# KorAP/Datok

Hardware: AMD Instinct MI355X
Metric: input MB/s tokenized, tokenizer_de.matok (higher is better)
Workload: dtype u32 table cells, u8 symbol codes; 1 GPU; tokenizer_de.matok, 4096 equal-length 4096 B synthetic German docs per batch (BASELINE.json configs[1]); table_layout=matrix: state-major fused u32 cells, docs_per_gpu=4096, doc_bytes=4096, parallelism=documents sharded over 1 GPU(s), no data-path collective, batches_in_flight=3, inputs=one per batch in flight (generator seeds 2, 3, 4 on rank 0)

## Files before the change

### datok_amd/csrc/dtk_walk.hip

```cpp
#include "dtk_walk_core.h"

struct ExactSink {
  DtkSymAt s;
  const uint8_t *txt;
  bool nl_rule, write;
  DtkCall *log;
  int32_t *rstart, *rend, *sent;
  uint32_t *bstart, *bend, *ttok, *tsent, *sbefore, *ts_end;
  uint32_t tok_n, sent_n, text_n;
  int32_t posC, last_rend;
  bool init, sentB;
  uint32_t n_tok, n_sent, n_text, n_sev, text_tok0, n_calls;
  uint32_t st;
  __device__ __forceinline__ void start() {
    posC = 0; last_rend = 0; init = true; sentB = true;
    n_tok = n_sent = n_text = n_sev = text_tok0 = n_calls = 0; st = 0;
  }
  __device__ __forceinline__ int32_t runes(uint32_t from, uint32_t to) const {
    return to > from ? (int32_t)count_runes(s, from, to) : 0;
  }
  __device__ __forceinline__ void call(uint32_t kind, int32_t a, uint32_t b, uint32_t c) {
    if (write) log[n_calls] = DtkCall{kind, a, b, c};
    n_calls++;
  }
  __device__ __forceinline__ void push_sent(int32_t v) {
    if (write) { if (n_sent < sent_n) sent[n_sent] = v; else st |= ST_INTERNAL; }
    n_sent++;
  }
  __device__ __forceinline__ void sentence_end(int32_t arg) {
    call(1u, arg, 0u, 0u);
    n_sev++;
    if (n_tok == text_tok0) st |= ST_EMPTY_TEXT; else push_sent(last_rend);
    sentB = true;
  }
  __device__ __forceinline__ void text_end(int32_t arg) {
    call(2u, arg, 0u, 0u);
    if (n_tok == text_tok0) st |= ST_EMPTY_TEXT;
    if (write) {
      if (n_text < text_n) {
        ttok[n_text] = n_tok; tsent[n_text] = n_sent;
        if (ts_end) ts_end[n_text] = n_sev;
      } else st |= ST_INTERNAL;
    }
    n_text++;
    sentB = true; posC = 0; text_tok0 = n_tok;
  }
  template <bool IS_MATRIX>
  __device__ __forceinline__ void token(uint32_t bs, uint32_t tp, uint32_t p, bool) {
    call(0u, (int32_t)bs, tp, p);
    const int32_t off_r = runes(bs, tp), len_r = runes(bs, p);
    if (posC == 0 && nl_rule && p > bs && txt[bs] == '\n' && !init) posC--;
    init = false;
    posC += off_r;
    const int32_t rs = posC;
    if (sentB) { sentB = false; push_sent(rs); }
    posC += len_r - off_r;
    last_rend = posC;
    if (write) {
      if (n_tok < tok_n) {
        if (rstart) { rstart[n_tok] = rs; rend[n_tok] = posC; }
        if (bstart) { bstart[n_tok] = tp < p ? tp : p; bend[n_tok] = p; }
        if (sbefore) sbefore[n_tok] = n_sev;
      } else st |= ST_INTERNAL;
    }
    n_tok++;
  }
  template <bool IS_MATRIX>
  __device__ __forceinline__ void eot(uint32_t bs, uint32_t p, bool with_sentence, bool) {
    const int32_t buffc = runes(bs, p);
    if (with_sentence) sentence_end(buffc);
    text_end(IS_MATRIX ? buffc : 0);
  }
  template <bool IS_MATRIX>
  __device__ __forceinline__ void sentence(uint32_t bs, uint32_t p, bool) {
    sentence_end(IS_MATRIX ? runes(bs, p) : 0);
  }
  template <bool IS_MATRIX>
  __device__ __forceinline__ void tail(uint32_t bs, uint32_t p, bool sentence_end_, bool text_end_, bool) {
    const int32_t arg = IS_MATRIX ? runes(bs, p) : 0;
    if (!sentence_end_) sentence_end(arg);
    if (!text_end_) text_end(arg);
  }
  __device__ __forceinline__ void out_of_order() {}
};

template <typename TRANS, bool IS_MATRIX>
__global__ __launch_bounds__(WAVE) void k_exact_doc(TRANS tr, DtkExactArgs X, uint32_t epsilon, uint32_t unknown,
                                                    uint32_t identity) {
  __shared__ uint16_t s_win[WAVE * DTK_WIN_ROW];
  uint16_t *win_row = s_win + threadIdx.x * DTK_WIN_ROW;
  const uint32_t i = blockIdx.x * WAVE + threadIdx.x;
  if (i >= X.n) return;
  const uint32_t d = X.docs[i];
  const uint64_t off = X.doc_off[d];
  const uint32_t len = (uint32_t)(X.doc_off[d + 1] - off);
  ExactSink sink;
  sink.s = DtkSymAt{X.sym, off}; sink.txt = X.text + off;
  sink.nl_rule = (X.flags & 16u) != 0; sink.write = X.pass != 0;
  sink.log = X.pass ? X.calls + X.call_off[i] : nullptr;
  const uint64_t t0 = X.tok_off[d], s0 = X.sent_off[d], x0 = X.text_off[d];
  sink.rstart = X.tok_rstart ? X.tok_rstart + t0 : nullptr; sink.rend = X.tok_rend ? X.tok_rend + t0 : nullptr;
  sink.bstart = X.tok_bstart ? X.tok_bstart + t0 : nullptr; sink.bend = X.tok_bend ? X.tok_bend + t0 : nullptr;
  sink.sbefore = X.tok_sbefore ? X.tok_sbefore + t0 : nullptr;
  sink.sent = X.sent + s0;
  sink.ttok = X.text_tok_end + x0; sink.tsent = X.text_sent_end + x0;
  sink.ts_end = X.text_s_end ? X.text_s_end + x0 : nullptr;
  sink.tok_n = (uint32_t)(X.tok_off[d + 1] - t0); sink.sent_n = (uint32_t)(X.sent_off[d + 1] - s0);
  sink.text_n = (uint32_t)(X.text_off[d + 1] - x0);
  sink.start();
  DtkLaneState init{0u, tr.start_state(), tr.start_aux(), 0u}, fin;
  uint32_t st = 0, steps = 0;
  walk_lane<TRANS, IS_MATRIX, MODE_DOC, ExactSink>(tr, X.sym, off, len, init, 0u, sink, epsilon, unknown, identity,
                                                   step_cap(X.step_factor, len), fin, st, steps, win_row);
  if (X.pass == 0) { X.n_calls[i] = sink.n_calls; return; }
  if (sink.n_tok != sink.tok_n || sink.n_sent != sink.sent_n || sink.n_text != sink.text_n) st |= ST_INTERNAL;
  X.status[d] = st | sink.st;
  if (X.doc_ns) X.doc_ns[d] = sink.n_sev;
}

template <typename TRANS, bool IS_MATRIX>
__global__ __launch_bounds__(WAVE) void k_walk_doc(TRANS tr, DtkWalkArgs A, uint32_t epsilon,
                                                   uint32_t unknown, uint32_t identity) {
  DTK_WINDOWS(TRANS, A.sym)
  const uint32_t d = blockIdx.x * WAVE + threadIdx.x;
  uint32_t steps = 0;
  if (d < A.n_docs) {
    const uint64_t off = A.doc_off[d];
    const uint32_t len = (uint32_t)(A.doc_off[d + 1] - off);
    EventSink sink;
    sink.init(A, off, d, 0u, 0xFFFFFFFFu);
    DtkLaneState init{0u, tr.start_state(), tr.start_aux(), 0u}, fin;
    uint32_t st;
    walk_any<TRANS, IS_MATRIX, MODE_DOC>(tr, A.sym, off, len, init, 0u, sink, epsilon, unknown,
                                          identity, step_cap(A.step_factor, len), fin, st, steps, win_row, s_lut);
    A.status[d] = st | sink.st;
    A.tok_cnt[d] = sink.c_tok; A.sent_cnt[d] = sink.c_sent; A.text_cnt[d] = sink.c_text;
  }
  add_steps(A.steps, steps);
}


#ifdef DTK_PROBE
__shared__ unsigned long long s_probe_mark;
__device__ unsigned long long g_phase[8];
extern "C" int dtk_phase_read(unsigned long long *out, int reset) {
  hipDeviceSynchronize();
  hipMemcpyFromSymbol(out, HIP_SYMBOL(g_phase), sizeof(g_phase));
  if (reset) { unsigned long long z[8] = {0}; hipMemcpyToSymbol(HIP_SYMBOL(g_phase), z, sizeof(z)); }
  return 0;
}
#endif

template <typename TRANS, bool IS_MATRIX>
__device__ __forceinline__ DtkLaneState start_record(const TRANS &tr, const DtkWalkArgs &A, const DtkSpecArgs &S,
                                                     uint32_t k, uint64_t off, uint32_t len, uint32_t epsilon,
                                                     uint32_t unknown, uint32_t identity, uint16_t *win_row,
                                                     const uint16_t *s_lut, uint32_t &steps) {
  DtkLaneState rec{0u, tr.start_state(), tr.start_aux(), 0u};
  if (k > 0) {
    const uint32_t kc = k * S.chunk;
    uint32_t sp = kc > S.warm ? kc - S.warm : 0u;
    if (sp > 0 && S.warm_extend && S.text) {
      const uint8_t *tx = S.text + off;
      auto load8 = [&](uint32_t q) -> uint64_t {
        if (off + q >= 16u) {
          const uint64_t a0 = reinterpret_cast<uint64_t>(tx + q) - 8u;
          const uint32_t sh = (uint32_t)(a0 & 3u) * 8u;
          const uint32_t *wp = reinterpret_cast<const uint32_t *>(a0 & ~3ull);
          const uint64_t lo64 = (uint64_t)wp[0] | ((uint64_t)wp[1] << 32);
          return sh ? (lo64 >> sh) | ((uint64_t)wp[2] << (64u - sh)) : lo64;
        }
        uint64_t w = 0;
        for (uint32_t k = 0; k < 8u; k++)
          if (q + k >= 8u) w |= (uint64_t)tx[q + k - 8u] << (8u * k);
        return w;
      };
      auto zb = [](uint64_t x) {
        return ~(((x & 0x7F7F7F7F7F7F7F7Full) + 0x7F7F7F7F7F7F7F7Full) | x) & 0x8080808080808080ull;
      };
      const uint32_t lim = sp > S.warm_extend ? sp - S.warm_extend : 0u;
      uint32_t q = sp;
      while (q > lim) {
        const uint64_t w = load8(q);
        uint64_t m = zb(w ^ 0x2020202020202020ull) | zb(w ^ 0x0A0A0A0A0A0A0A0Aull) |
                     zb(w ^ 0x0909090909090909ull) | zb(w ^ 0x0D0D0D0D0D0D0D0Dull);
        if (q < 8u) m &= ~0ull << ((8u - q) * 8u);
        if (m) {
          q = q - 8u + (7u - ((uint32_t)__clzll((long long)m) >> 3)) + 1u;
          break;
        }
        q = q >= 8u ? q - 8u : 0u;
      }
      if (q < lim) q = lim;
      sp = q;
      uint64_t wt[DTK_WARM_TAG / 8u];
#pragma unroll
      for (uint32_t i = 0; i < DTK_WARM_TAG / 8u; i++) wt[i] = sp > 8u * i ? load8(sp - 8u * i) : 0ull;
#pragma unroll
      for (uint32_t i = 0; i < DTK_WARM_TAG / 8u; i++) {
        const uint32_t qq = sp > 8u * i ? sp - 8u * i : 0u;
        uint64_t mo = zb(wt[i] ^ 0x3C3C3C3C3C3C3C3Cull), mc = zb(wt[i] ^ 0x3E3E3E3E3E3E3E3Eull);
        if (qq < 8u) { const uint64_t in = qq ? ~0ull << ((8u - qq) * 8u) : 0ull; mo &= in; mc &= in; }
        if (mo | mc) {
          if (mo > mc) sp = qq - 8u + (7u - ((uint32_t)__clzll((long long)mo) >> 3));
          break;
        }
      }
    }
#ifdef DTK_PROBE
    s_probe_mark = clock64();
#endif
    EventSink sink;
    sink.g = nullptr; sink.lds = (dtk_lds_u32 *)nullptr; sink.tailw = nullptr; sink.lw = 0; sink.lo = sink.hi = 0;
    uint32_t st;
    if (sp > 0) {
      while (sp < len && !dtk_sym_is_start(A.sym, off + sp)) sp++;
      DtkLaneState init{sp, tr.start_state(), tr.start_aux(), 0u};
      walk_any<TRANS, IS_MATRIX, MODE_START>(tr, A.sym, off, len, init, kc, sink, epsilon, unknown,
                                              identity, step_cap(A.step_factor, len), rec, st, steps, win_row, s_lut);
    } else {
      walk_any<TRANS, IS_MATRIX, MODE_START>(tr, A.sym, off, len, rec, kc, sink, epsilon, unknown,
                                              identity, step_cap(A.step_factor, len), rec, st, steps, win_row, s_lut);
    }
  }
  return rec;
}

template <typename TRANS, bool IS_MATRIX>
__global__ __launch_bounds__(WAVE) void k_spec_start(TRANS tr, DtkWalkArgs A, DtkSpecArgs S,
                                                     uint32_t epsilon, uint32_t unknown,
                                                     uint32_t identity) {
  DTK_WINDOWS(TRANS, A.sym)
  const uint32_t L = blockIdx.x * WAVE + threadIdx.x;
  uint32_t steps = 0;
  if (L < S.n_lanes) {
    const uint32_t d = S.lane_doc[L];
    const uint32_t k = L - S.chunk_off[d];
    const uint64_t off = A.doc_off[d];
    const uint32_t len = (uint32_t)(A.doc_off[d + 1] - off);
    S.lane_start[L] = start_record<TRANS, IS_MATRIX>(tr, A, S, k, off, len, epsilon, unknown, identity, win_row, s_lut, steps);
  }
  add_steps(A.steps, steps);
}

extern __shared__ uint32_t s_dyn_bits[];

#ifndef DTK_WALK_OCC
#define DTK_WALK_OCC 7
#endif
template <typename TRANS, bool IS_MATRIX>
__global__ __launch_bounds__(WAVE, TRANS::LEAN ? DTK_WALK_OCC : 1) void k_spec_both(TRANS tr, DtkWalkArgs A, DtkSpecArgs S,
                                                    uint32_t epsilon, uint32_t unknown,
                                                    uint32_t identity) {
  DTK_WINDOWS(TRANS, A.sym)
  uint32_t *lds_bits = S.lds_words ? s_dyn_bits : nullptr;
#ifdef DTK_PROBE
  const unsigned long long pt0 = clock64();
  unsigned long long pt1 = pt0, pt2 = pt0;
  s_probe_mark = pt0;
#endif
  const uint32_t L = blockIdx.x * WAVE + threadIdx.x;
  const uint32_t w0 = S.lds_words ? lds_bits_word0(A, S, blockIdx.x * WAVE) : 0u;
  if (lds_bits) lds_bits_clear(lds_bits, S.lds_words);
  uint32_t steps = 0;
  if (L < S.n_lanes) {
    const uint32_t d = S.lane_doc[L];
    const uint32_t k = L - S.chunk_off[d];
    const uint64_t off = A.doc_off[d];
    const uint32_t len = (uint32_t)(A.doc_off[d + 1] - off);
    const DtkLaneState rec =
        start_record<TRANS, IS_MATRIX>(tr, A, S, k, off, len, epsilon, unknown, identity, win_row, s_lut, steps);
#ifdef DTK_PROBE
    pt1 = clock64();
#endif
    S.lane_start[L] = rec;
    DtkLaneState fin{0xFFFFFFFFu, 0u, 0u, LANE_F_IDLE};
    DtkLaneCount cnt{0u, 0u, 0u, 0u, 0u, 0xFFFFFFFFu, 0u, 0u};
    const uint32_t stop = (L + 1u < S.chunk_off[d + 1]) ? (k + 1u) * S.chunk : 0xFFFFFFFFu;
    if (rec.p != 0xFFFFFFFFu && rec.p >= stop) {
      fin = rec;
      fin.flags &= (LANE_F_SENT | LANE_F_TEXT | LANE_F_OK);
    } else if (rec.p != 0xFFFFFFFFu) {
      EventSink sink;
      sink.init(A, off, d, rec.p, 0xFFFFFFFFu, lds_bits, S.lds_words, w0);
      uint32_t st = 0, steps2 = 0;
      walk_any<TRANS, IS_MATRIX, MODE_CHUNK, true>(tr, A.sym, off, len, rec, stop, sink, epsilon, unknown,
                                                    identity, step_cap(A.step_factor, len), fin, st, steps2, win_row, s_lut);
      steps += steps2;
      if (sink.dropped) fin.flags |= LANE_F_DROPPED;
      cnt.tok = sink.c_tok; cnt.sent = sink.c_sent; cnt.text = sink.c_text; cnt.status = st | sink.st;
      cnt.sev = sink.c_sev; cnt.e_pos = sink.e_pos; cnt.e_tok = sink.e_tok;
    }
#ifdef DTK_PROBE
    pt2 = clock64();
#endif
    S.lane_end[L] = fin;
    S.lane_cnt[L] = cnt;
  }
  if (lds_bits) lds_bits_flush(lds_bits, S.lds_words, A.bits, A.bit_words, w0);
  add_steps(A.steps, steps);
#ifdef DTK_PROBE
  {
    __syncthreads();
    const unsigned long long pt3 = clock64(), mark = s_probe_mark;
    if (threadIdx.x == 0) {
      atomicAdd(&g_phase[0], mark - pt0); atomicAdd(&g_phase[1], pt1 - mark); atomicAdd(&g_phase[2], pt2 - pt1);
      atomicAdd(&g_phase[3], pt3 - pt2); atomicAdd(&g_phase[4], 1ull);
    }
  }
#endif
}

__device__ __forceinline__ DtkLanePlan plan_of(const DtkSpecArgs &S, uint32_t L, uint32_t d) {
  const uint32_t L0 = S.chunk_off[d], L1 = S.chunk_off[d + 1];
  const uint32_t k = L - L0, fb = ~S.first_bad[d];
  DtkLanePlan pl;
  pl.pad = 0;
  if (k < fb) {
    pl.stop = pl.wend = S.lane_start[L + 1].p;
    pl.mode = PLAN_CHAINED;
  } else if (k == fb) {
    pl.stop = (L + 1 < L1) ? (k + 1u) * S.chunk : 0xFFFFFFFFu;
    pl.wend = 0xFFFFFFFFu;
    pl.mode = PLAN_LAST;
  } else {
    pl.stop = pl.wend = 0;
    pl.mode = PLAN_OFF;
  }
  return pl;
}

template <typename TRANS, bool IS_MATRIX>
__global__ __launch_bounds__(WAVE) void k_spec_walk(TRANS tr, DtkWalkArgs A, DtkSpecArgs S,
                                                    uint32_t epsilon, uint32_t unknown,
                                                    uint32_t identity) {
  DTK_WINDOWS(TRANS, A.sym)
  if (S.go && *S.go == 0u) return;
  uint32_t *lds_bits = S.lds_words ? s_dyn_bits : nullptr;
  const uint32_t L = blockIdx.x * WAVE + threadIdx.x;
  const uint32_t w0 = S.lds_words ? lds_bits_word0(A, S, blockIdx.x * WAVE) : 0u;
  if (lds_bits) lds_bits_clear(lds_bits, S.lds_words);
  uint32_t steps = 0;
  if (L < S.n_lanes) {
    const uint32_t d = S.lane_doc[L];
    const bool redo = S.redo_from != nullptr;
    if (!redo || (S.redo_from[d] != 0xFFFFFFFFu && L >= S.redo_from[d])) {
      const DtkLanePlan pl = plan_of(S, L, d);
      DtkLaneState fin{0xFFFFFFFFu, 0u, 0u, LANE_F_IDLE};
      DtkLaneCount cnt{0u, 0u, 0u, 0u, 0u, 0xFFFFFFFFu, 0u, 0u};
      const DtkLaneState init0 = pl.mode == PLAN_CHAINED ? S.lane_start[L] : DtkLaneState{0xFFFFFFFFu, 0u, 0u, 0u};
      if (pl.mode == PLAN_CHAINED && init0.p != 0xFFFFFFFFu && init0.p >= pl.stop) {
        fin = init0;
        fin.flags &= (LANE_F_SENT | LANE_F_TEXT | LANE_F_OK);
      } else if (pl.mode != PLAN_OFF) {
        const uint64_t off = A.doc_off[d];
        const uint32_t len = (uint32_t)(A.doc_off[d + 1] - off);
        const DtkLaneState init = S.lane_start[L];
        EventSink sink;
        sink.init(A, off, d, init.p, pl.wend, lds_bits, S.lds_words, w0);
        uint32_t st = 0;
        walk_any<TRANS, IS_MATRIX, MODE_CHUNK>(tr, A.sym, off, len, init, pl.stop, sink, epsilon, unknown,
                                                identity, step_cap(A.step_factor, len), fin, st, steps, win_row, s_lut);
        if (sink.dropped) fin.flags |= LANE_F_DROPPED;
        cnt.tok = sink.c_tok; cnt.sent = sink.c_sent; cnt.text = sink.c_text; cnt.status = st | sink.st;
        cnt.sev = sink.c_sev; cnt.e_pos = sink.e_pos; cnt.e_tok = sink.e_tok;
      }
      S.lane_end[L] = fin;
      S.lane_cnt[L] = cnt;
    }
  }
  if (lds_bits) lds_bits_flush(lds_bits, S.lds_words, A.bits, A.bit_words, w0);
  add_steps(A.steps, steps);
}


extern "C" int dtk_launch_walk(const DtkTableDev *tab, const DtkWalkArgs *args, void *stream) {
  if (args->n_docs == 0) return 0;
  const uint32_t blocks = (args->n_docs + WAVE - 1) / WAVE;
  hipStream_t s = (hipStream_t)stream;
  return with_trans(tab, args->sym.lut != nullptr, [&](auto tr, auto is_matrix) {
    using TR = decltype(tr);
    hipLaunchKernelGGL((k_walk_doc<TR, decltype(is_matrix)::value>), dim3(blocks), dim3(WAVE), 0, s, tr, *args,
                       tab->epsilon, tab->unknown, tab->identity);
  });
}

extern "C" int dtk_launch_spec(const DtkTableDev *tab, const DtkWalkArgs *args, const DtkSpecArgs *spec,
                               int stage, uint32_t cmp_mask, uint32_t *redo_out, uint32_t *n_bad,
                               void *stream) {
  if (args->n_docs == 0 || spec->n_lanes == 0) return 0;
  hipStream_t s = (hipStream_t)stream;
  const uint32_t lane_blocks = (spec->n_lanes + WAVE - 1) / WAVE;
  switch (stage) {
    case 0:
      return with_trans(tab, args->sym.lut != nullptr, [&](auto tr, auto is_matrix) {
        using TR = decltype(tr);
        hipLaunchKernelGGL((k_spec_start<TR, decltype(is_matrix)::value>), dim3(lane_blocks), dim3(WAVE), 0, s,
                           tr, *args, *spec, tab->epsilon, tab->unknown, tab->identity);
      });
    case 6:
      return with_trans(tab, args->sym.lut != nullptr, [&](auto tr, auto is_matrix) {
        using TR = decltype(tr);
        hipLaunchKernelGGL((k_spec_both<TR, decltype(is_matrix)::value>), dim3(lane_blocks), dim3(WAVE),
                           3u * spec->lds_words * sizeof(uint32_t), s, tr, *args, *spec, tab->epsilon, tab->unknown,
                           tab->identity);
      });
    case 2:
      return with_trans(tab, args->sym.lut != nullptr, [&](auto tr, auto is_matrix) {
        using TR = decltype(tr);
        hipLaunchKernelGGL((k_spec_walk<TR, decltype(is_matrix)::value>), dim3(lane_blocks), dim3(WAVE),
                           3u * spec->lds_words * sizeof(uint32_t), s, tr, *args, *spec, tab->epsilon, tab->unknown,
                           tab->identity);
      });
    case 1: case 3: case 7: case 4: case 5:
      return dtk_launch_spec_check(args, spec, stage, cmp_mask, redo_out, n_bad, stream);
  }
  return -1;
}

extern "C" int dtk_launch_exact(const DtkTableDev *tab, const DtkExactArgs *args, void *stream) {
  if (args->n == 0) return 0;
  const uint32_t blocks = (args->n + WAVE - 1) / WAVE;
  hipStream_t s = (hipStream_t)stream;
  return with_trans(tab, args->sym.lut != nullptr, [&](auto tr, auto is_matrix) {
    using TR = decltype(tr);
    if constexpr (TR::LEAN) {
      const typename TR::general base = tr;
      hipLaunchKernelGGL((k_exact_doc<typename TR::general, decltype(is_matrix)::value>), dim3(blocks), dim3(WAVE), 0, s, base, *args,
                         tab->epsilon, tab->unknown, tab->identity);
    } else {
      hipLaunchKernelGGL((k_exact_doc<TR, decltype(is_matrix)::value>), dim3(blocks), dim3(WAVE), 0, s, tr, *args,
                         tab->epsilon, tab->unknown, tab->identity);
    }
  });
}
```

### datok_amd/csrc/dtk_walk_core.h

```cpp
#pragma once
#include "dtk_device.h"


template <typename CELL>
struct MatrixTrans {
  const CELL *tab;
  uint32_t stride, n_eps, start;
  static constexpr CELL FLAG = (CELL)((CELL)1 << (sizeof(CELL) * 8 - 1));
  static constexpr bool FUSED = false;
  static constexpr bool LEAN = false;
  __device__ __forceinline__ uint32_t start_state() const { return start; }
  __device__ __forceinline__ uint32_t start_aux() const { return 0; }
  __device__ __forceinline__ bool has_eps(uint32_t t, uint32_t) const { return t <= n_eps; }
  __device__ __forceinline__ bool step(uint32_t t0, uint32_t, uint32_t a, uint32_t &t,
                                       uint32_t &aux, bool &nontoken, uint32_t &st, uint32_t &via) const {
    via = 0;
    const CELL x = tab[(size_t)t0 * stride + a];
    t = (uint32_t)(x & (CELL)~FLAG);
    nontoken = (x & FLAG) != 0;
    aux = 0;
    (void)st;
    return t != 0;
  }
};
// ... 173 lines not shown
    put_first(EVB_SEPS, p);
  }
  template <bool IS_MATRIX>
  __device__ __forceinline__ void tail_(uint32_t p, bool sentence_end, bool text_end, bool has_tok) {
    const uint32_t bits = (sentence_end ? 0u : DTK_TAIL_S) | (text_end ? 0u : DTK_TAIL_E);
    if (!bits) return;
    if (!in_opening(p)) { dropped = 1; return; }
    if (!text_end) c_text++;
    c_sev += sentence_end ? 0u : 1u;
    if (has_tok) c_sent += sentence_end ? 0u : 1u; else st |= ST_EMPTY_TEXT;
    if (tailw) *tailw = (p << 2) | bits;
  }
  template <bool IS_MATRIX>
  __device__ __forceinline__ void tail(uint32_t , uint32_t p, bool sentence_end, bool text_end, bool has_tok) {
    tail_<IS_MATRIX>(p, sentence_end, text_end, has_tok);
  }
  __device__ __forceinline__ void out_of_order() { st |= ST_IRREGULAR; }
  __device__ __forceinline__ void flush() {}
};

__device__ __forceinline__ void lds_bits_clear(uint32_t *lds_, uint32_t lw) {
  dtk_lds_u32 *lds = (dtk_lds_u32 *)lds_;
  for (uint32_t j = threadIdx.x; j < 3u * lw; j += WAVE) lds[j] = 0u;
  __syncthreads();
}
__device__ __forceinline__ void lds_bits_flush(const uint32_t *lds_, uint32_t lw, uint32_t *g, uint32_t gw, uint32_t w0) {
  const dtk_lds_u32 *lds = (const dtk_lds_u32 *)lds_;
  __syncthreads();
  for (uint32_t j = threadIdx.x; j < lw; j += WAVE) {
    if (w0 + j >= gw) break;
#pragma unroll
    for (uint32_t k = 0; k < 3u; k++) {
      const uint32_t v = lds[k * lw + j];
      if (v) atomicOr(&g[k * gw + w0 + j], v);
    }
  }
}
__device__ __forceinline__ uint32_t lds_bits_word0(const DtkWalkArgs &A, const DtkSpecArgs &S, uint32_t L0) {
  const uint32_t d0 = S.lane_doc[L0];
  return (uint32_t)((DTK_EV_BIT(A.doc_off[d0], d0) + (uint64_t)(L0 - S.chunk_off[d0]) * S.chunk) >> 5);
}

template <typename TRANS>
__device__ __forceinline__ uint32_t guard_of(const TRANS &tr) {
  if constexpr (TRANS::FUSED) return tr.ident_guard; else return 0xFFFFFFFFu;
}

enum { MODE_DOC = 0,
       MODE_START = 1,
       MODE_CHUNK = 2
};

struct DtkSymAt { DtkSym S; uint64_t off; };
__device__ __noinline__ uint32_t count_runes(const DtkSymAt &s, uint32_t from, uint32_t to) {
  uint32_t n = 0;
  for (uint32_t i = from; i < to; i++) n += dtk_sym_is_start(s.S, s.off + i) ? 1u : 0u;
  return n;
}

typedef uint2 __attribute__((may_alias)) dtk_u2a;
typedef uint16_t __attribute__((may_alias)) dtk_u16a;
typedef uint8_t __attribute__((may_alias)) dtk_u8a;
__device__ __forceinline__ void win_fill(dtk_u16a *row, const DtkSym &S, uint64_t at) {
  if (S.lut) {
    const uint2 *__restrict__ g = reinterpret_cast<const uint2 *>(static_cast<const uint8_t *>(S.base) + at);
    uint2 c[DTK_WIN / 8u];
#pragma unroll
    for (uint32_t i = 0; i < DTK_WIN / 8u; i++) c[i] = g[i];
    dtk_u2a *r = reinterpret_cast<dtk_u2a *>(row);
#pragma unroll
    for (uint32_t i = 0; i < DTK_WIN / 8u; i++) {
      const uint32_t lo = c[i].x, hi = c[i].y;
      r[2 * i] = make_uint2((uint32_t)S.lut[lo & 255u] | ((uint32_t)S.lut[(lo >> 8) & 255u] << 16),
                            (uint32_t)S.lut[(lo >> 16) & 255u] | ((uint32_t)S.lut[lo >> 24] << 16));
      r[2 * i + 1] = make_uint2((uint32_t)S.lut[hi & 255u] | ((uint32_t)S.lut[(hi >> 8) & 255u] << 16),
                                (uint32_t)S.lut[(hi >> 16) & 255u] | ((uint32_t)S.lut[hi >> 24] << 16));
    }
    return;
  }
  const uint4 *__restrict__ g = reinterpret_cast<const uint4 *>(static_cast<const uint16_t *>(S.base) + at);
  uint4 v[DTK_WIN / 8u];
#pragma unroll
  for (uint32_t i = 0; i < DTK_WIN / 8u; i++) v[i] = g[i];
  dtk_u2a *r = reinterpret_cast<dtk_u2a *>(row);
#pragma unroll
  for (uint32_t i = 0; i < DTK_WIN / 8u; i++) {
    r[2 * i] = make_uint2(v[i].x, v[i].y);
    r[2 * i + 1] = make_uint2(v[i].z, v[i].w);
  }
}

__device__ __forceinline__ void win_fill8(dtk_u8a *row, const uint8_t *__restrict__ from) {
  const uint4 *__restrict__ g = reinterpret_cast<const uint4 *>(from);
  uint4 v[DTK_WIN8 / 16u];
#pragma unroll
  for (uint32_t i = 0; i < DTK_WIN8 / 16u; i++) v[i] = g[i];
  dtk_u2a *r = reinterpret_cast<dtk_u2a *>(row);
#pragma unroll
  for (uint32_t i = 0; i < DTK_WIN8 / 16u; i++) {
    r[2 * i] = make_uint2(v[i].x, v[i].y);
    r[2 * i + 1] = make_uint2(v[i].z, v[i].w);
  }
}

template <typename TRANS, bool IS_MATRIX, int MODE, typename SINK = EventSink>
__device__ __forceinline__ void walk_lane(const TRANS &tr, const DtkSym &sym,
                                          uint64_t off, uint32_t len, DtkLaneState init, uint32_t stop_pos,
                                          SINK &sink, uint32_t epsilon, uint32_t unknown,
                                          uint32_t identity, uint32_t cap, DtkLaneState &fin,
                                          uint32_t &st_out, uint32_t &steps_out, uint16_t *win_row) {
  dtk_u16a *row = reinterpret_cast<dtk_u16a *>(win_row);
  const uint32_t o7 = (uint32_t)(off & 7u);
  const uint64_t aligned = off - o7;
  const DtkSymAt s{sym, off};

  uint32_t a = 0, t0 = 0, aux0 = 0;
  uint32_t t = init.t, aux = init.aux;
  const uint32_t t_start = tr.start_state(), aux_start = tr.start_aux();
  bool ok = (init.flags & LANE_F_OK) != 0;
  uint32_t eps_t = 0, eps_aux = 0, eps_p = 0;
  bool sentence_end = (init.flags & LANE_F_SENT) != 0, text_end = (init.flags & LANE_F_TEXT) != 0;
  uint32_t p = init.p;
  uint32_t tp = init.p;
  uint32_t bs = init.p;
  uint32_t hi = init.p;
  uint32_t w = 1;
  bool eot = false, newchar = true;
  uint32_t st = 0, my_steps = 0;
  fin.p = 0xFFFFFFFFu; fin.t = 0; fin.aux = 0; fin.flags = 0;
  bool stopped = false;
  bool any_tok = init.p > 0;
  bool has_tok = init.p > 0 && !text_end;

  uint32_t wbase = (init.p + o7) & ~7u;
  win_fill(row, sym, aligned + wbase);

  bool done = false;
  do {
    if (newchar && p >= len) {
      const bool he = tr.has_eps(t, aux);
      const bool bt = !he && eps_t != 0;
      t0 = bt ? eps_t : t; aux0 = bt ? eps_aux : aux;
      p = bt ? eps_p : p;
      eps_t = bt ? 0u : eps_t;
      a = epsilon;
      newchar = false;
      done = !he && !bt;
    }
    if (__builtin_amdgcn_ballot_w64(newchar && (p + o7 - wbase) >= DTK_WIN) != 0ull) {
      wbase = (p + o7) & ~7u;
      win_fill(row, sym, aligned + wbase);
    }
    if (newchar) {
      const uint32_t e = row[p + o7 - wbase];
      a = e & DTK_SYM_MASK;
      w = DTK_SYM_WIDTH(e);
      const uint32_t cls = (e >> DTK_SYM_CLS_SHIFT) & 3u;
      hi = max(hi, p + w);
      eot = cls == 1u;
      ok = cls >= 2u ? cls == 2u : ok;
      t0 = t; aux0 = aux;
      const bool he = tr.has_eps(t0, aux0);
      eps_t = he ? t0 : eps_t; eps_aux = he ? aux0 : eps_aux;
      eps_p = he ? p : eps_p;
    }

    bool nontoken = false;
    uint32_t via = 0;
    const bool fresh = newchar;
    bool good = tr.step(t0, aux0, a, t, aux, nontoken, st, via);
    const bool act = !done;
    my_steps += act ? 1u : 0u;
    const bool is_eps = a == epsilon;
    bool comp = false;
    if (TRANS::FUSED) {
      comp = act && good && via != 0 && fresh && !(!ok && a == guard_of(tr)) &&
             !(MODE != MODE_DOC && p >= stop_pos);
      good = good && (via == 0 || comp);
    }
    const bool succ = act && good && !comp, fail = act && !good;
    const bool retry_unknown = fail && !ok && a == identity;
    const bool backtrack = fail && !retry_unknown && !is_eps && eps_t != 0;
    bool hardfail = fail && !retry_unknown && !backtrack;
    const bool flush_eps = succ && is_eps && p > tp;
    const bool sent_eps = succ && is_eps && p <= tp;
    const bool advance = succ && !is_eps;
    const bool eot_now = (succ || comp) && eot;

    if (hardfail || my_steps > cap) {
      if (hardfail) {
        if (is_eps) { st |= ST_BAD_MODEL; done = true; hardfail = false; }
        else if (p <= tp) { p += w; }
        if (hardfail && p < tp) st |= ST_BAD_OFFSET;
        t = t_start; aux = aux_start;
      }
      if (my_steps > cap) { st |= ST_STEP_LIMIT; done = true; hardfail = false; }
    }
    const bool flush_c = comp && p > tp, sent_c = comp && p <= tp;
    const bool flush = flush_eps || hardfail || flush_c;
    if (MODE != MODE_START) {
      if (flush)
        sink.template token<IS_MATRIX>(bs, tp, p, sentence_end || text_end || !any_tok);
      if (sent_eps || sent_c) sink.template sentence<IS_MATRIX>(bs, p, has_tok);
    }
    any_tok = any_tok || flush;
    has_tok = has_tok || flush;
    const bool skip = (advance && p == tp && nontoken) || (comp && nontoken && p >= tp);
    const uint32_t p_old = p;
    p = (advance || comp) ? p + w : p;
    tp = skip ? p : (flush_c ? p_old : tp);
    const bool eot_sent = !((flush_c || flush_eps) ? false : ((sent_c || sent_eps) ? true : sentence_end));
    sentence_end = eot_now ? true : (flush ? false : ((sent_eps || sent_c) ? true : sentence_end));
    text_end = eot_now ? true : (flush ? false : text_end);
    t0 = backtrack ? eps_t : t0; aux0 = backtrack ? eps_aux : aux0;
    p = backtrack ? eps_p : p;
    a = backtrack ? epsilon : (retry_unknown ? unknown : a);
    eot = (retry_unknown || backtrack) ? false : eot;
    newchar = succ || hardfail || comp;
    eot = eot_now ? false : eot;
    const bool rewind = flush || (IS_MATRIX && eot_now);
    eps_t = (backtrack || rewind || comp) ? 0u : eps_t;
    if (TRANS::FUSED) {
      const bool he2 = comp && !(IS_MATRIX && eot_now) && tr.has_eps(via, 0u);
      eps_t = he2 ? via : eps_t; eps_p = he2 ? p_old : eps_p;
    }
    const bool rewind_end = (flush && !comp) || (IS_MATRIX && eot_now);
    const bool long_win = hi - bs > DTK_WINDOW_BYTES;
    const bool at_stop = rewind_end && MODE != MODE_DOC && p >= stop_pos && !(hardfail && eot && p >= len);
    if (eot_now || (rewind && hi - bs > DTK_WINDOW) || at_stop || long_win) {
      if (eot_now) {
        if (is_eps && MODE != MODE_START) sink.out_of_order();
        if (MODE != MODE_START) sink.template eot<IS_MATRIX>(flush_c ? p_old : bs, p, eot_sent, has_tok);
        has_tok = false;
      }
      if (rewind) {
        if (hi - bs > DTK_WINDOW && count_runes(s, bs, hi) > DTK_WINDOW) st |= ST_WINDOW_OVERFLOW;
        if (at_stop) {
          fin.p = p; fin.t = t; fin.aux = aux;
          fin.flags = (sentence_end ? LANE_F_SENT : 0u) | (text_end ? LANE_F_TEXT : 0u) |
                      (ok ? LANE_F_OK : 0u);
          stopped = true;
          done = true;
        }
      }
      if (long_win && !done) { st |= ST_WINDOW_OVERFLOW; done = true; }
    }
    tp = rewind_end ? p : tp;
    bs = rewind_end ? p : (flush_c ? p_old : bs);
  } while (!done);

  if (!stopped && !(st & (ST_STEP_LIMIT | ST_BAD_MODEL))) {
    if (hi - bs > DTK_WINDOW && count_runes(s, bs, hi) > DTK_WINDOW) st |= ST_WINDOW_OVERFLOW;
    if (MODE != MODE_START) {
      if (p > tp) {
        sink.template token<IS_MATRIX>(bs, tp, p, sentence_end || text_end || !any_tok);
        sentence_end = false; text_end = false;
        has_tok = true;
      }
      sink.template tail<IS_MATRIX>(bs, p, sentence_end, text_end, has_tok);
    }
  }
  st_out = st;
  steps_out = my_steps;
}

#ifdef DTK_PROBE
__device__ unsigned long long g_probe[8];
extern "C" int dtk_probe_read(unsigned long long *out, int reset) {
  hipDeviceSynchronize();
  hipMemcpyFromSymbol(out, HIP_SYMBOL(g_probe), sizeof(g_probe));
  if (reset) { unsigned long long z[8] = {0}; hipMemcpyToSymbol(HIP_SYMBOL(g_probe), z, sizeof(z)); }
  return 0;
}
#endif

template <int MODE, bool FIRST = false, bool IS_MATRIX = true, typename TRANS = MatrixFusedTrans>
__device__ __forceinline__ void walk_fused(const TRANS &tr, const DtkSym &sym,
                                           uint64_t off, uint32_t len, DtkLaneState init, uint32_t stop_pos,
                                           EventSink &sink, uint32_t epsilon, uint32_t cap, DtkLaneState &fin,
                                           uint32_t &st_out, uint32_t &steps_out, uint16_t *win_row,
                                           const uint16_t *lut) {
  typedef typename TRANS::cell CELL;
  typedef typename CELL::raw cell_t;
  const DtkSymAt s{sym, off};
  const cell_t *__restrict__ tab = tr.tab;
  const uint32_t stride = tr.stride, n_eps = tr.n_eps;
  uint32_t t = init.t;
  uint32_t p = init.p, tp = init.p, bs = init.p, hi = init.p;
  uint32_t eps_t = 0, eps_p = 0;
  uint32_t F = (init.flags & (LANE_F_SENT | LANE_F_TEXT)) | (init.p > 0 ? 4u : 0u);
  F |= (init.p > 0 && !(init.flags & LANE_F_TEXT)) ? 8u : 0u;
  static_assert(LANE_F_SENT == 1u && LANE_F_TEXT == 2u, "flag layout");
  uint32_t st = 0;
  uint32_t budget = cap;
  fin.p = 0xFFFFFFFFu; fin.t = 0; fin.aux = 0; fin.flags = 0;
  bool done = false;
  dtk_u8a *row = reinterpret_cast<dtk_u8a *>(win_row);
  const uint32_t o7 = (uint32_t)(off & 15u);
  const uint8_t *__restrict__ aligned = static_cast<const uint8_t *>(sym.base) + (off - o7);
#define DTK_ENTRY(q_) ((uint32_t)lut[row[(q_) - wb7]])
#define DTK_REFILL(q_) { wb7 = (((q_) + o7) & ~15u) - o7; win_fill8(row, aligned + (wb7 + o7)); }
  uint32_t wb7;
  DTK_REFILL(p)
  uint32_t e = DTK_ENTRY(p);

  auto eof_drain = [&](const bool eot_stale) __attribute__((always_inline)) {
    if (p >= len) {
      bool first_ = true;
      while (t <= n_eps && !done) {
        const cell_t x_ = tab[__umul24(t, stride) + epsilon];
        const bool ov_ = __builtin_usub_overflow(budget, 1u, &budget);
        if ((int32_t)CELL::head(x_) <= 0) { st |= ST_BAD_MODEL; done = true; break; }
        if (p > tp) {
          if (MODE != MODE_START) sink.template token<IS_MATRIX>(bs, tp, p, ((F ^ 4u) & 7u) != 0);
          F = 12u;
          if (hi - bs > DTK_WINDOW && count_runes(s, bs, hi) > DTK_WINDOW) st |= ST_WINDOW_OVERFLOW;
          tp = p; bs = p; eps_t = 0;
          if (MODE != MODE_DOC && p >= stop_pos) {
            fin.p = p; fin.t = CELL::target(x_); fin.aux = 0; fin.flags = init.flags & LANE_F_OK;
            done = true;
          }
        } else {
          if (MODE != MODE_START) sink.template sentence<IS_MATRIX>(bs, p, (F & 8u) != 0);
          F |= 1u;
        }
        t = CELL::target(x_);
        if (eot_stale && first_ && !done) {
          if (MODE != MODE_START) sink.out_of_order();
          if (MODE != MODE_START) sink.template eot<IS_MATRIX>(bs, p, (F & 1u) == 0u, (F & 8u) != 0);
          F = (F & 4u) | 3u;
          if (IS_MATRIX) {
            eps_t = 0; tp = p; bs = p;
            if (MODE != MODE_DOC && p >= stop_pos) {
              fin.p = p; fin.t = t; fin.aux = 0; fin.flags = (F & 3u) | (init.flags & LANE_F_OK);
              done = true;
            }
          }
        }
        first_ = false;
        if (ov_) { st |= ST_STEP_LIMIT; done = true; }
      }
      if (!done) {
        if (eps_t != 0) { t = eps_t; p = eps_p; eps_t = 0; e = epsilon; } else done = true;
      }
    }
  };
  eof_drain(false);
  cell_t x = CELL::none();
  uint32_t en = 0;
#define DTK_TAB(t_, e_) (*reinterpret_cast<const cell_t *>(reinterpret_cast<const char *>(tab) +                    \
                                                          ((__umul24((t_), stride) + ((e_) & DTK_SYM_MASK)) << CELL::SHIFT)))
  if (!done) {
    x = DTK_TAB(t, e);
    const uint32_t pn0 = p + ((e >> DTK_SYM_W_SHIFT) & 7u);
    if (pn0 - wb7 >= DTK_WIN8) DTK_REFILL(pn0)
    en = DTK_ENTRY(pn0);
  }
#ifdef DTK_PROBE
  unsigned long long pr_wait = 0, pr_t0 = clock64(), pr_n = 0, pr_refill = 0, pr_nrefill = 0;
#endif
  while (!done) {
    const bool over = __builtin_usub_overflow(budget, 1u, &budget);
    const uint32_t w = (e >> DTK_SYM_W_SHIFT) & 7u;
    const uint32_t pn = p + w;
    const bool he = t <= n_eps;
    eps_t = he ? t : eps_t; eps_p = he ? p : eps_p;
    const bool r = w == 0u;
    const uint32_t xh = CELL::head(x);
    const uint32_t tgt = CELL::target(x), via = CELL::via(x);
    const bool comp = (int32_t)xh < 0;
    const bool plain = (int32_t)xh > 0;
    const bool fail = xh == 0u;
    const bool advance = comp || (plain && !r);
    const bool backtrack = fail && !r && eps_t != 0;
    const uint32_t t_n = backtrack ? eps_t : (fail ? t : tgt);
    const uint32_t p_n = backtrack ? eps_p : (advance ? pn : p);
    const uint32_t e_n = backtrack ? epsilon : en;
    const cell_t x_n = DTK_TAB(t_n, e_n);
    const unsigned long long m_comp = __builtin_amdgcn_ballot_w64((int32_t)xh < 0),
                             m_adv = m_comp | (__builtin_amdgcn_ballot_w64((int32_t)xh > 0) & ~__builtin_amdgcn_ballot_w64(w == 0u));
    const unsigned long long m_skip = __builtin_amdgcn_ballot_w64(CELL::nontoken(x)) &
                                      ((m_comp & __builtin_amdgcn_ballot_w64(p > tp)) | (m_adv & __builtin_amdgcn_ballot_w64(p == tp)));
    uint32_t code_n;
    {
      const uint32_t pn_n = p_n + ((e_n >> DTK_SYM_W_SHIFT) & 7u);
      uint32_t iw = pn_n - wb7;
      if (__builtin_amdgcn_ballot_w64(iw >= DTK_WIN8) != 0ull) {
#ifdef DTK_PROBE
        const unsigned long long r0_ = clock64();
#endif
        DTK_REFILL(pn_n)
        iw = pn_n - wb7;
#ifdef DTK_PROBE
        asm volatile("s_waitcnt vmcnt(0) lgkmcnt(0)" ::: "memory");
        pr_refill += clock64() - r0_;
        pr_nrefill++;
#endif
      }
      code_n = row[iw];
    }
    hi = max(hi, pn);
    const bool epsE = comp || (plain && r);
    const bool flush = epsE && p > tp;
    const bool sentE = epsE && p <= tp;
    const bool hardfail = fail && !backtrack;
    const bool beyond = MODE != MODE_DOC && p >= stop_pos;
    const uint32_t tp_old = tp, F_old = F;
    if (MODE != MODE_START) {
      if (FIRST) {
        if (flush && !beyond) sink.template token_first<IS_MATRIX>(tp, p, ((F ^ 4u) & 7u) != 0);
        if (sentE && !beyond) sink.sentence_first(p, (F & 8u) != 0);
      } else {
        if (flush) sink.template token<IS_MATRIX>(bs, tp, p, ((F ^ 4u) & 7u) != 0);
        if (sentE) sink.template sentence<IS_MATRIX>(bs, p, (F & 8u) != 0);
      }
    }
    const uint32_t win = hi - bs;
    const uint32_t bs_old = bs, p_old = p;
    F = flush ? 12u : (F | (sentE ? 1u : 0u));
    bs = flush ? p_old : bs;

    tp = flush ? p_old : tp;
    tp = __builtin_amdgcn_inverse_ballot_w64(m_skip) ? pn : tp;
    const bool he2 = comp && via <= n_eps;
    eps_t = he2 ? via : ((backtrack || epsE) ? 0u : eps_t);
    eps_p = he2 ? p_old : eps_p;
    const uint32_t e_cur = e, e_next = en;
    p = p_n; t = t_n; e = e_n; x = x_n; en = lut[code_n];
    const bool eot_now = advance && ((e_cur >> DTK_SYM_CLS_SHIFT) & 3u) == 1u;
    const bool at_stop = flush && beyond;
    if (hardfail | eot_now | (beyond & (FIRST ? epsE : flush)) | (flush & (win > DTK_WINDOW)) | (win > DTK_WINDOW_BYTES) |
        over | ((p >= len) & !backtrack)) {
      if (FIRST && MODE != MODE_START && beyond) {
        if (flush) sink.template token<IS_MATRIX>(bs_old, tp_old, p_old, ((F_old ^ 4u) & 7u) != 0);
        if (sentE) sink.template sentence<IS_MATRIX>(bs_old, p_old, (F_old & 8u) != 0);
      }
      if (flush && win > DTK_WINDOW && count_runes(s, bs_old, hi) > DTK_WINDOW) st |= ST_WINDOW_OVERFLOW;
      bool eot_stale = false;
      if (at_stop) {
        fin.p = p_old; fin.t = comp ? via : tgt; fin.aux = 0;
        fin.flags = init.flags & LANE_F_OK;
        done = true;
      } else {
        if (hardfail) {
          if (r) { st |= ST_BAD_MODEL; done = true; }
          else {
            if (p <= tp) { p = pn; }
            if (p < tp) st |= ST_BAD_OFFSET;
            e = p == pn ? e_next : e_cur;
            eot_stale = p == pn && p >= len && ((e_cur >> DTK_SYM_CLS_SHIFT) & 3u) == 1u;
            if (MODE != MODE_START) sink.template token<IS_MATRIX>(bs, tp, p, ((F ^ 4u) & 7u) != 0);
            F = 12u;
            if (hi - bs > DTK_WINDOW && count_runes(s, bs, hi) > DTK_WINDOW) st |= ST_WINDOW_OVERFLOW;
            t = tr.start; eps_t = 0;
            tp = p; bs = p;
            if (MODE != MODE_DOC && p >= stop_pos && !eot_stale) {
              fin.p = p; fin.t = t; fin.aux = 0;
              fin.flags = (init.flags & LANE_F_OK);
              done = true;
            }
          }
        }
        if (eot_now) {
          if (MODE != MODE_START) sink.template eot<IS_MATRIX>(bs, p, (F & 1u) == 0u, (F & 8u) != 0);
          F = (F & 4u) | 3u;
          if (IS_MATRIX) {
            eps_t = 0;
            if (hi - bs > DTK_WINDOW && count_runes(s, bs, hi) > DTK_WINDOW) st |= ST_WINDOW_OVERFLOW;
            tp = p; bs = p;
            if (MODE != MODE_DOC && p >= stop_pos && !done) {
              fin.p = p; fin.t = t; fin.aux = 0;
              fin.flags = (F & 3u) | (init.flags & LANE_F_OK);
              done = true;
            }
          }
        }
        if (over && !done) { st |= ST_STEP_LIMIT; done = true; }
        if (hi - bs > DTK_WINDOW_BYTES && !done) { st |= ST_WINDOW_OVERFLOW; done = true; }
      }
      if (!done && !backtrack) eof_drain(eot_stale);
      if (!done) {
        x = DTK_TAB(t, e);
        const uint32_t pn2 = p + ((e >> DTK_SYM_W_SHIFT) & 7u);
        if (pn2 - wb7 >= DTK_WIN8) DTK_REFILL(pn2)
        en = DTK_ENTRY(pn2);
      }
    }
#ifdef DTK_PROBE
    {
      const unsigned long long a_ = clock64();
      asm volatile("s_waitcnt vmcnt(0) lgkmcnt(0)" ::: "memory");
      pr_wait += clock64() - a_;
      pr_n++;
    }
#endif
  }
#undef DTK_TAB
#undef DTK_ENTRY
#undef DTK_REFILL
#ifdef DTK_PROBE
  {
    const unsigned long long tot_ = clock64() - pr_t0;
    unsigned long long wmax = pr_wait, nmax = pr_n;
    for (int o = 32; o; o >>= 1) {
      const unsigned long long a_ = __shfl_xor(wmax, o), b_ = __shfl_xor(nmax, o);
      wmax = a_ > wmax ? a_ : wmax; nmax = b_ > nmax ? b_ : nmax;
    }
    if (MODE == MODE_CHUNK && lane_id() == 0) {
      atomicAdd(&g_probe[0], wmax); atomicAdd(&g_probe[1], tot_); atomicAdd(&g_probe[2], nmax); atomicAdd(&g_probe[3], 1ull);
    }
    if (MODE == MODE_CHUNK && lane_id() == 0) {
      atomicAdd(&g_probe[4], pr_refill); atomicAdd(&g_probe[5], pr_nrefill);
    }
  }
#endif

  if (fin.p == 0xFFFFFFFFu && !(st & (ST_STEP_LIMIT | ST_BAD_MODEL))) {
    if (hi - bs > DTK_WINDOW && count_runes(s, bs, hi) > DTK_WINDOW) st |= ST_WINDOW_OVERFLOW;
    if (MODE != MODE_START) {
      if (p > tp) {
        sink.template token<IS_MATRIX>(bs, tp, p, ((F ^ 4u) & 7u) != 0);
        F = (F & ~3u) | 8u;
      }
      sink.template tail<IS_MATRIX>(bs, p, (F & 1u) != 0, (F & 2u) != 0, (F & 8u) != 0);
    }
  }
  st_out = st;
  steps_out = cap - budget;
}

template <typename TRANS, bool IS_MATRIX, int MODE, bool FIRST = false>
__device__ __forceinline__ void walk_any(const TRANS &tr, const DtkSym &sym, uint64_t off,
                                         uint32_t len, DtkLaneState init, uint32_t stop_pos, EventSink &sink,
                                         uint32_t epsilon, uint32_t unknown, uint32_t identity, uint32_t cap,
                                         DtkLaneState &fin, uint32_t &st_out, uint32_t &steps_out,
                                         uint16_t *win_row, const uint16_t *lut) {
  if constexpr (TRANS::LEAN)
    walk_fused<MODE, FIRST, IS_MATRIX, TRANS>(tr, sym, off, len, init, stop_pos, sink, epsilon, cap, fin, st_out, steps_out, win_row, lut);
  else
    walk_lane<TRANS, IS_MATRIX, MODE>(tr, sym, off, len, init, stop_pos, sink, epsilon, unknown, identity, cap,
                                      fin, st_out, steps_out, win_row);
}

__device__ __forceinline__ uint32_t step_cap(uint32_t factor, uint32_t len) {
  unsigned long long c = (unsigned long long)factor * ((unsigned long long)len + 2ull);
  return c > 0xFFFFFFF0ull ? 0xFFFFFFF0u : (uint32_t)c;
}

__device__ __forceinline__ void add_steps(unsigned long long *counter, uint32_t mine) {
  unsigned long long tot = mine;
#pragma unroll
  for (int o = 32; o > 0; o >>= 1) tot += __shfl_down(tot, o);
  if (lane_id() == 0 && tot) atomicAdd(counter + (blockIdx.x & (DTK_STEP_STRIPES - 1u)) * 16u, tot);
}

#ifndef DTK_ROW_PAD
#define DTK_ROW_PAD 0u
#endif
#define DTK_WINDOWS(TRANS, SYM)                                                                       \
  constexpr uint32_t WIN_ROW_ = TRANS::LEAN ? (DTK_WIN8 + DTK_ROW_PAD) / 2u : DTK_WIN_ROW;            \
  __shared__ uint16_t s_win[WAVE * WIN_ROW_];                                                         \
  __shared__ uint16_t s_lut[TRANS::LEAN ? 256 : 1];                                                   \
  uint16_t *win_row = s_win + threadIdx.x * WIN_ROW_;                                                 \
  if constexpr (TRANS::LEAN) {                                                                        \
    for (uint32_t i_ = threadIdx.x; i_ < 256u; i_ += WAVE) s_lut[i_] = (SYM).lut[i_];                 \
    __syncthreads();                                                                                  \
  }

template <typename F>
static int with_trans(const DtkTableDev *tab, bool codes, F &&f) {
  if (tab->kind == DTK_KIND_MATRIX) {
    if (tab->fused) {
      auto call = [&](auto t) { if (tab->da_dense) f(t, std::false_type{}); else f(t, std::true_type{}); };
      auto pick = [&](auto gen, auto lean) {
        gen.tab = (decltype(gen.tab))tab->tab;
        gen.stride = tab->stride; gen.n_eps = tab->n_eps; gen.start = tab->start; gen.ident_guard = tab->ident_guard;
        if (tab->ident_guard == 0xFFFFFFFFu && codes) {
          static_cast<decltype(gen) &>(lean) = gen;
          call(lean);
        } else {
          call(gen);
        }
      };
      if (tab->entry_bytes == 8) pick(MatrixFused64Trans{}, MatrixLean64Trans{});
      else pick(MatrixFusedTrans{}, MatrixLeanTrans{});
    } else if (tab->entry_bytes == 2) {
      MatrixTrans<uint16_t> tr{(const uint16_t *)tab->tab, tab->stride, tab->n_eps, tab->start};
      f(tr, std::true_type{});
    } else {
      MatrixTrans<uint32_t> tr{(const uint32_t *)tab->tab, tab->stride, tab->n_eps, tab->start};
      f(tr, std::true_type{});
    }
  } else {
    DaTrans tr{(const uint2 *)tab->tab, tab->da_len, tab->da_size, tab->da_base1};
    f(tr, std::false_type{});
  }
  return (int)hipGetLastError();
}
```

Measured before the change: 170,900 MB/s.

## Vectorize warm-start scan with bulk 16-byte loads and overlap LUT fetch with lane setup

Measured after the change: 174,800 MB/s (median of 6 runs). 1.02x the previous value.

```diff
diff --git a/datok_amd/csrc/dtk_walk.hip b/datok_amd/csrc/dtk_walk.hip
--- a/datok_amd/csrc/dtk_walk.hip
+++ b/datok_amd/csrc/dtk_walk.hip
@@ -151,6 +151,51 @@
 }
 #endif
 
+#ifndef DTK_WARM_STRETCH
+#define DTK_WARM_STRETCH 112u
+#endif
+static_assert(DTK_WARM_STRETCH % 16u == 0 && DTK_WARM_STRETCH >= DTK_WARM_TAG + 16u && DTK_WARM_TAG % 8u == 0, "stretch layout");
+
+__device__ __forceinline__ uint64_t zero_bytes(uint64_t x) {
+  return ~(((x & 0x7F7F7F7F7F7F7F7Full) + 0x7F7F7F7F7F7F7F7Full) | x) & 0x8080808080808080ull;
+}
+__device__ __forceinline__ uint64_t blank_bytes(uint64_t w) {
+  return zero_bytes(w ^ 0x2020202020202020ull) | zero_bytes(w ^ 0x0A0A0A0A0A0A0A0Aull) |
+         zero_bytes(w ^ 0x0909090909090909ull) | zero_bytes(w ^ 0x0D0D0D0D0D0D0D0Dull);
+}
+__device__ __forceinline__ uint64_t bracket_bytes(uint64_t w) {
+  return zero_bytes((w | 0x0202020202020202ull) ^ 0x3E3E3E3E3E3E3E3Eull);
+}
+__device__ __forceinline__ uint32_t top_byte(uint64_t m) {
+  return 7u - ((uint32_t)__clzll((long long)m) >> 3);
+}
+
+typedef const uint8_t __attribute__((address_space(1))) dtk_glb_u8;
+typedef const uint64_t __attribute__((address_space(1), aligned(1), may_alias)) dtk_glb_u64u;
+__device__ __noinline__ uint32_t warm_start_far(const uint8_t *text_, uint64_t off, uint32_t q, uint32_t lim) {
+  dtk_glb_u8 *text = (dtk_glb_u8 *)text_;
+  auto load8 = [&](uint32_t q_) -> uint64_t {
+    uint64_t w = 0;
+    if (q_ >= 8u) w = *(dtk_glb_u64u *)(text + (off + q_ - 8u));
+    else for (uint32_t i = 0; i < q_; i++) w |= (uint64_t)text[off + i] << (8u * (8u - q_ + i));
+    return w;
+  };
+  while (q > lim) {
+    const uint64_t m = blank_bytes(load8(q));
+    if (m) { q = q - 8u + top_byte(m) + 1u; break; }
+    q = q >= 8u ? q - 8u : 0u;
+  }
+  if (q < lim) q = lim;
+  for (uint32_t qq = q, i = 0; qq > 0u && i < DTK_WARM_TAG / 8u; qq = qq >= 8u ? qq - 8u : 0u, i++) {
+    const uint64_t w = load8(qq), m = bracket_bytes(w);
+    if (m) {
+      const uint32_t j = top_byte(m);
+      return ((w >> (8u * j)) & 2u) ? q : qq - 8u + j;
+    }
+  }
+  return q;
+}
+
 template <typename TRANS, bool IS_MATRIX>
 __device__ __forceinline__ DtkLaneState start_record(const TRANS &tr, const DtkWalkArgs &A, const DtkSpecArgs &S,
                                                      uint32_t k, uint64_t off, uint32_t len, uint32_t epsilon,
@@ -161,49 +206,66 @@
     const uint32_t kc = k * S.chunk;
     uint32_t sp = kc > S.warm ? kc - S.warm : 0u;
     if (sp > 0 && S.warm_extend && S.text) {
-      const uint8_t *tx = S.text + off;
-      auto load8 = [&](uint32_t q) -> uint64_t {
-        if (off + q >= 16u) {
-          const uint64_t a0 = reinterpret_cast<uint64_t>(tx + q) - 8u;
-          const uint32_t sh = (uint32_t)(a0 & 3u) * 8u;
-          const uint32_t *wp = reinterpret_cast<const uint32_t *>(a0 & ~3ull);
-          const uint64_t lo64 = (uint64_t)wp[0] | ((uint64_t)wp[1] << 32);
-          return sh ? (lo64 >> sh) | ((uint64_t)wp[2] << (64u - sh)) : lo64;
+      const uint32_t lim = sp > S.warm_extend ? sp - S.warm_extend : 0u;
+      if (off + sp < DTK_WARM_STRETCH) {
+        sp = warm_start_far(S.text, off, sp, lim);
+      } else {
+        constexpr uint32_t NW = DTK_WARM_STRETCH / 8u, NB = (DTK_WARM_STRETCH - DTK_WARM_TAG) / 8u;
+        uint64_t w[NW];
+        {
+          const uint8_t *__restrict__ from = S.text + (off + sp - DTK_WARM_STRETCH);
+          uint4 v[NW / 2u];
+#pragma unroll
+          for (uint32_t i = 0; i < NW / 2u; i++) __builtin_memcpy(&v[i], from + 16u * i, 16);
+#pragma unroll
+          for (uint32_t i = 0; i < NW / 2u; i++) {
+            w[2 * i] = (uint64_t)v[i].x | ((uint64_t)v[i].y << 32);
+            w[2 * i + 1] = (uint64_t)v[i].z | ((uint64_t)v[i].w << 32);
+          }
         }
-        uint64_t w = 0;
-        for (uint32_t k = 0; k < 8u; k++)
-          if (q + k >= 8u) w |= (uint64_t)tx[q + k - 8u] << (8u * k);
-        return w;
-      };
-      auto zb = [](uint64_t x) {
-        return ~(((x & 0x7F7F7F7F7F7F7F7Full) + 0x7F7F7F7F7F7F7F7Full) | x) & 0x8080808080808080ull;
-      };
-      const uint32_t lim = sp > S.warm_extend ? sp - S.warm_extend : 0u;
-      uint32_t q = sp;
-      while (q > lim) {
-        const uint64_t w = load8(q);
-        uint64_t m = zb(w ^ 0x2020202020202020ull) | zb(w ^ 0x0A0A0A0A0A0A0A0Aull) |
-                     zb(w ^ 0x0909090909090909ull) | zb(w ^ 0x0D0D0D0D0D0D0D0Dull);
-        if (q < 8u) m &= ~0ull << ((8u - q) * 8u);
-        if (m) {
-          q = q - 8u + (7u - ((uint32_t)__clzll((long long)m) >> 3)) + 1u;
-          break;
+        const uint32_t sp0 = sp;
+        uint32_t q = sp;
+        bool found = false;
+#pragma unroll
+        for (uint32_t j = NW; j-- > NW - NB;) {
+          if (!found && q > lim) {
+            uint64_t m = blank_bytes(w[j]);
+            if (q < 8u) m &= ~0ull << ((8u - q) * 8u);
+            found = m != 0ull;
+            q = found ? q - 8u + top_byte(m) + 1u : (q >= 8u ? q - 8u : 0u);
+          }
         }
-        q = q >= 8u ? q - 8u : 0u;
-      }
-      if (q < lim) q = lim;
-      sp = q;
-      uint64_t wt[DTK_WARM_TAG / 8u];
+        if (!found && q > lim) {
+          sp = warm_start_far(S.text, off, q, lim);
+        } else {
+          if (q < lim) q = lim;
+          uint64_t any = 0;
 #pragma unroll
-      for (uint32_t i = 0; i < DTK_WARM_TAG / 8u; i++) wt[i] = sp > 8u * i ? load8(sp - 8u * i) : 0ull;
+          for (uint32_t j = 0; j < NW; j++) {
+            const uint64_t x = (w[j] | 0x0202020202020202ull) ^ 0x3E3E3E3E3E3E3E3Eull;
+            any |= (x - 0x0101010101010101ull) & ~x;
+          }
+          sp = q;
+          if (any & 0x8080808080808080ull) {
+            uint64_t bm = 0, bw = 0;
+            uint32_t back = 0;
 #pragma unroll
-      for (uint32_t i = 0; i < DTK_WARM_TAG / 8u; i++) {
-        const uint32_t qq = sp > 8u * i ? sp - 8u * i : 0u;
-        uint64_t mo = zb(wt[i] ^ 0x3C3C3C3C3C3C3C3Cull), mc = zb(wt[i] ^ 0x3E3E3E3E3E3E3E3Eull);
-        if (qq < 8u) { const uint64_t in = qq ? ~0ull << ((8u - qq) * 8u) : 0ull; mo &= in; mc &= in; }
-        if (mo | mc) {
-          if (mo > mc) sp = qq - 8u + (7u - ((uint32_t)__clzll((long long)mo) >> 3));
-          break;
+            for (uint32_t j = NW; j-- > 0u;) {
+              if (bm == 0ull) {
+                uint64_t m = bracket_bytes(w[j]);
+                if (j >= NW - NB) {
+                  const int32_t keep = (int32_t)(q - sp0) + (int32_t)(8u * (NW - j));
+                  m = keep <= 0 ? 0ull : (keep < 8 ? m & ~(~0ull << (8 * keep)) : m);
+                }
+                bm = m; bw = w[j]; back = 8u * (NW - j);
+              }
+            }
+            if (bm) {
+              const uint32_t j = top_byte(bm);
+              const int64_t at = (int64_t)sp0 - (int64_t)back + (int64_t)j;
+              if (at >= 0 && at + (int64_t)DTK_WARM_TAG >= (int64_t)q && !((bw >> (8u * j)) & 2u)) sp = (uint32_t)at;
+            }
+          }
         }
       }
     }
@@ -214,7 +276,7 @@
     sink.g = nullptr; sink.lds = (dtk_lds_u32 *)nullptr; sink.tailw = nullptr; sink.lw = 0; sink.lo = sink.hi = 0;
     uint32_t st;
     if (sp > 0) {
-      while (sp < len && !dtk_sym_is_start(A.sym, off + sp)) sp++;
+      if constexpr (!TRANS::LEAN) while (sp < len && !dtk_sym_is_start(A.sym, off + sp)) sp++;
       DtkLaneState init{sp, tr.start_state(), tr.start_aux(), 0u};
       walk_any<TRANS, IS_MATRIX, MODE_START>(tr, A.sym, off, len, init, kc, sink, epsilon, unknown,
                                               identity, step_cap(A.step_factor, len), rec, st, steps, win_row, s_lut);
@@ -230,11 +292,13 @@
 __global__ __launch_bounds__(WAVE) void k_spec_start(TRANS tr, DtkWalkArgs A, DtkSpecArgs S,
                                                      uint32_t epsilon, uint32_t unknown,
                                                      uint32_t identity) {
-  DTK_WINDOWS(TRANS, A.sym)
+  DTK_WINDOWS_DECL(TRANS)
   const uint32_t L = blockIdx.x * WAVE + threadIdx.x;
+  const uint2 lut4 = lut_request<TRANS>(A.sym);
+  const uint32_t d = S.lane_doc[min(L, S.n_lanes - 1u)];
+  lut_store<TRANS>(s_lut, lut4);
   uint32_t steps = 0;
   if (L < S.n_lanes) {
-    const uint32_t d = S.lane_doc[L];
     const uint32_t k = L - S.chunk_off[d];
     const uint64_t off = A.doc_off[d];
     const uint32_t len = (uint32_t)(A.doc_off[d + 1] - off);
@@ -252,7 +316,7 @@
 __global__ __launch_bounds__(WAVE, TRANS::LEAN ? DTK_WALK_OCC : 1) void k_spec_both(TRANS tr, DtkWalkArgs A, DtkSpecArgs S,
                                                     uint32_t epsilon, uint32_t unknown,
                                                     uint32_t identity) {
-  DTK_WINDOWS(TRANS, A.sym)
+  DTK_WINDOWS_DECL(TRANS)
   uint32_t *lds_bits = S.lds_words ? s_dyn_bits : nullptr;
 #ifdef DTK_PROBE
   const unsigned long long pt0 = clock64();
@@ -260,14 +324,17 @@
   s_probe_mark = pt0;
 #endif
   const uint32_t L = blockIdx.x * WAVE + threadIdx.x;
-  const uint32_t w0 = S.lds_words ? lds_bits_word0(A, S, blockIdx.x * WAVE) : 0u;
+  const uint2 lut4 = lut_request<TRANS>(A.sym);
+  const uint32_t d = S.lane_doc[min(L, S.n_lanes - 1u)];
+  lut_store<TRANS>(s_lut, lut4);
   if (lds_bits) lds_bits_clear(lds_bits, S.lds_words);
+  const uint32_t k = L - S.chunk_off[d];
+  const uint64_t off = A.doc_off[d];
+  const uint32_t len = (uint32_t)(A.doc_off[d + 1] - off);
+  const bool last = L + 1u >= S.chunk_off[d + 1];
+  const uint32_t w0 = S.lds_words ? __builtin_amdgcn_readfirstlane((uint32_t)((DTK_EV_BIT(off, d) + (uint64_t)k * S.chunk) >> 5)) : 0u;
   uint32_t steps = 0;
   if (L < S.n_lanes) {
-    const uint32_t d = S.lane_doc[L];
-    const uint32_t k = L - S.chunk_off[d];
-    const uint64_t off = A.doc_off[d];
-    const uint32_t len = (uint32_t)(A.doc_off[d + 1] - off);
     const DtkLaneState rec =
         start_record<TRANS, IS_MATRIX>(tr, A, S, k, off, len, epsilon, unknown, identity, win_row, s_lut, steps);
 #ifdef DTK_PROBE
@@ -276,7 +343,7 @@
     S.lane_start[L] = rec;
     DtkLaneState fin{0xFFFFFFFFu, 0u, 0u, LANE_F_IDLE};
     DtkLaneCount cnt{0u, 0u, 0u, 0u, 0u, 0xFFFFFFFFu, 0u, 0u};
-    const uint32_t stop = (L + 1u < S.chunk_off[d + 1]) ? (k + 1u) * S.chunk : 0xFFFFFFFFu;
+    const uint32_t stop = last ? 0xFFFFFFFFu : (k + 1u) * S.chunk;
     if (rec.p != 0xFFFFFFFFu && rec.p >= stop) {
       fin = rec;
       fin.flags &= (LANE_F_SENT | LANE_F_TEXT | LANE_F_OK);
diff --git a/datok_amd/csrc/dtk_walk_core.h b/datok_amd/csrc/dtk_walk_core.h
--- a/datok_amd/csrc/dtk_walk_core.h
+++ b/datok_amd/csrc/dtk_walk_core.h
@@ -499,6 +499,10 @@
 #define DTK_REFILL(q_) { wb7 = (((q_) + o7) & ~15u) - o7; win_fill8(row, aligned + (wb7 + o7)); }
   uint32_t wb7;
   DTK_REFILL(p)
+  if (MODE == MODE_START) {
+    while (p < len && p - wb7 < DTK_WIN8 && row[p - wb7] == DTK_SYM_CONT) p++;
+    tp = p; bs = p; hi = p;
+  }
   uint32_t e = DTK_ENTRY(p);
 
   auto eof_drain = [&](const bool eot_stale) __attribute__((always_inline)) {
@@ -754,15 +758,26 @@
 #ifndef DTK_ROW_PAD
 #define DTK_ROW_PAD 0u
 #endif
-#define DTK_WINDOWS(TRANS, SYM)                                                                       \
+#define DTK_WINDOWS_DECL(TRANS)                                                                       \
   constexpr uint32_t WIN_ROW_ = TRANS::LEAN ? (DTK_WIN8 + DTK_ROW_PAD) / 2u : DTK_WIN_ROW;            \
   __shared__ uint16_t s_win[WAVE * WIN_ROW_];                                                         \
-  __shared__ uint16_t s_lut[TRANS::LEAN ? 256 : 1];                                                   \
-  uint16_t *win_row = s_win + threadIdx.x * WIN_ROW_;                                                 \
-  if constexpr (TRANS::LEAN) {                                                                        \
-    for (uint32_t i_ = threadIdx.x; i_ < 256u; i_ += WAVE) s_lut[i_] = (SYM).lut[i_];                 \
-    __syncthreads();                                                                                  \
-  }
+  __shared__ __attribute__((aligned(8))) uint16_t s_lut[TRANS::LEAN ? 256 : 1];                       \
+  uint16_t *win_row = s_win + threadIdx.x * WIN_ROW_;
+template <typename TRANS>
+__device__ __forceinline__ uint2 lut_request(const DtkSym &sym) {
+  if constexpr (TRANS::LEAN) return reinterpret_cast<const uint2 *>(sym.lut)[threadIdx.x];
+  else return make_uint2(0u, 0u);
+}
+template <typename TRANS>
+__device__ __forceinline__ void lut_store(uint16_t *s_lut, uint2 v) {
+  if constexpr (TRANS::LEAN) {
+    reinterpret_cast<dtk_u2a *>(s_lut)[threadIdx.x] = v;
+    __syncthreads();
+  }
+}
+#define DTK_WINDOWS(TRANS, SYM)                                                                       \
+  DTK_WINDOWS_DECL(TRANS)                                                                             \
+  lut_store<TRANS>(s_lut, lut_request<TRANS>(SYM));
 
 template <typename F>
 static int with_trans(const DtkTableDev *tab, bool codes, F &&f) {
```
